# jserv/nstack

Hardware: AMD Instinct MI355X
Metric: device-resident CRC-32 FCS GiB/s on 1518-B frames, 1/2/4/8 MI355X; % HBM peak (higher is better)
Workload: dtype u8

## Files before the change

nstack_amd/csrc/fcs_engine.cpp:

```cpp
#include <hip/hip_runtime.h>

#include <algorithm>
#include <atomic>
#include <cerrno>
#include <cstdarg>
#include <cstdio>
#include <cstdlib>
#include <chrono>
#include <cstring>
#include <map>
#include <memory>
#include <mutex>
#include <set>
#include <string>
#include <thread>
#include <vector>
#include <initializer_list>

#include "../../include/nstack_fcs.h"
#include "fcs_device.hpp"
#include "fcs_error.hpp"
#include "fcs_host_crc.hpp"
#include "fcs_launch.hpp"
#include "fcs_tables.hpp"
// ... 1447 lines not shown
    if (ds->tx_flag) hipHostFree(ds->tx_flag);
    if (ds->tx_dcount) hipFree(ds->tx_dcount);
    if (ds->vz_off) hipHostFree(ds->vz_off);
    if (ds->vz_len) hipHostFree(ds->vz_len);
    if (ds->vz_ok) hipHostFree(ds->vz_ok);
    if (ds->vz_dbad) hipFree(ds->vz_dbad);
    if (ds->one_stream) hipStreamDestroy(ds->one_stream);
    if (ds->one_h) hipHostFree(ds->one_h);
    if (ds->one_hout) hipHostFree(ds->one_hout);
    if (ds->one_flag) hipHostFree(ds->one_flag);
    for (DevState::OneLane &L : ds->one_lane) {
        if (L.st) hipStreamDestroy(L.st);
        if (L.flag) hipHostFree(L.flag);
    }
    if (!ds->q_streams.empty() || !ds->q_host.empty() || !ds->q_dev.empty()) (void)device_sync();
    for (hipStream_t q : ds->q_streams) hipStreamDestroy(q);
    for (void *h : ds->q_host) hipHostFree(h);
    for (void *d : ds->q_dev) hipFree(d);
    for (hipEvent_t ev : ds->ctr_done)
        if (ev) hipEventDestroy(ev);
    if (ds->d_blob) hipFree(ds->d_blob);
    if (ds->d_one_blob) hipFree(ds->d_one_blob);
    if (ds->d_kinit) hipFree(ds->d_kinit);
    if (ds->d_ctr) hipFree(ds->d_ctr);
    for (uint32_t *scr : ds->ctr_scr)
        if (scr) hipFree(scr);
}

extern "C" {

const char *fcs_last_error(void) { return g_last_error.c_str(); }

const char *fcs_engine_version(void) {
    return "nstack-fcs 0.6 gfx950: quarter-wave/frame, 96B lane windows as 2 slice-by-4 chains, v_perm "
           "addressing, DPP reduce; 1496-1524B: LDS-DMA (nt global_load_lds) 6KiB slot/wave, 16 waves/CU, "
           "32KiB 8-replica tables, guided dynamic items; 130-399B: 4 lanes x 36-104B, 400-868B: 8 lanes x 44-112B windows/frame, 870-1476B: 16 lanes x 60-96B windows, 6-7KiB LDS-DMA slots; <=128B: lane/frame; 1477-1495B, 1525-1988B: 104/120/128B-window LDS-DMA, 7/8KiB slots; "
           ">1524B otherwise: frame-interleaved LDS-DMA segments of 900-1988B (least m*(WD+8)); var: "
           "packed 64-1536B units as an arena stream (4KiB LDS-DMA items, taps at frame boundaries, XOR "
           "scan), other units as a flat chunk stream per 64-frame window";
}

int fcs_engine_init(int ndev) {
    int total = 0;
    hipError_t e = hipGetDeviceCount(&total);
    if (e != hipSuccess || total <= 0) return fail(ENODEV, "no HIP device visible (%s)", hipGetErrorString(e));
    const int use = ndev <= 0 ? total : ((ndev > total && !alias_devices_enabled()) ? total : ndev);
    {
        std::lock_guard<std::mutex> lk(g_mu);
        g_engine_devs.clear();
        for (int d = 0; d < use; d++) g_engine_devs.push_back(d);
        for (auto it = g_alias.begin(); it != g_alias.end();) {
            if (it->first >= use) {
                g_alias_retired.push_back(std::move(it->second));
                it = g_alias.erase(it);
            } else {
                ++it;
            }
        }
    }
    std::vector<DevState *> devs;
    int rc = engine_devices(&devs);
    if (rc) return rc;
    return use;
}

void fcs_engine_fini(void) {
    std::lock_guard<std::mutex> lk(g_mu);
    int cur = 0;
    (void)hipGetDevice(&cur);
    for (auto &up : g_dev)
        if (up) destroy_state(up.get());
    for (auto &kv : g_alias)
// ... 447 lines not shown
```

nstack_amd/csrc/fcs_kernel.hip:

```cpp
#include <hip/hip_runtime.h>
#include <stdint.h>

#include <atomic>

#include "dispenser.hpp"
#include "fcs_launch.hpp"
#include "fcs_tables.hpp"
#include "fcs_crc.hpp"
#include "wave_sync.hpp"

namespace fcs {

struct Item {
    uint64_t end;
    uint32_t len;
    uint32_t m;
};

template <bool VAR>
__device__ __forceinline__ Item frame_item(const KParams &p, uint64_t f) {
    Item it;
    if (VAR) {
        const uint32_t L = p.len[f];
        it.end = p.base + (p.off ? p.off[f] : f * p.stride) + L;
// ... 1514 lines not shown
#ifdef FCS_SHORT_NO_PIPE
    constexpr bool kPipe = false;
#else
    constexpr bool kPipe = W <= 24;
#endif
    if constexpr (!kPipe) {
        for (uint64_t it = D.first(); it != kEnd; it = D.next(it)) {
            Win x;
            load(it, x);
            crc(it, x);
        }
    } else {
    Win xa, xb;
    uint64_t it = D.first();
    if (it != kEnd) load(it, xa);
    while (it != kEnd) {
        const uint64_t i1 = D.next(it);
        if (i1 != kEnd) load(i1, xb);
        crc(it, xa);
        if (i1 == kEnd) break;
        const uint64_t i2 = D.next(i1);
        if (i2 != kEnd) load(i2, xa);
        crc(i1, xb);
        it = i2;
    }
    }
    flush_bad<kWideBad>(p, lds);
}

constexpr uint32_t kStChunk = 64;
constexpr uint32_t kStItem = 64 * kStChunk;
constexpr uint32_t kStSlotBytes = kStItem;
constexpr int kStWaves = kWgThreads / 64;
constexpr uint32_t kStHoleChunk = 0;
constexpr uint32_t kStHoleWord = kStHoleChunk + 4 * kStChunkTabs;
constexpr uint32_t kStHoleInv = kStHoleWord + 4 * kStWordTabs;
constexpr uint32_t kStHoleK1 = kStHoleInv + 4 * kStInvTabs;
constexpr uint32_t kStHoleMark = kStHoleK1 + 2;
constexpr uint32_t kStBad = dma_hole(kStHoleMark + 2 * 16);
static_assert(kStHoleMark + 2 * 16 + 1 <= 256, "holes");
static_assert(kStWaves <= 16, "marks and counters for 16 waves");
constexpr uint32_t kStSlots = 65536;
constexpr uint32_t kStRings = kStSlots + 16 * kStSlotBytes;
constexpr uint32_t kStLdsBytes = kStRings + 16 * 1024;
static_assert(kStLdsBytes <= 163840, "LDS per CU");
constexpr uint32_t kMarkStart = 1u << 31, kMarkEnd = 1u << 30;
constexpr uint32_t kStLenBits = 11;
static_assert(kStUnitFrames * kStMaxLen + 128 < (1u << (32 - kStLenBits)) && kStMaxLen < (1u << kStLenBits), "packing");
#ifdef FCS_STAMPS
#define ST_T(v)                              \
    __builtin_amdgcn_sched_barrier(0);       \
    const uint64_t v = __builtin_amdgcn_s_memtime(); \
    __builtin_amdgcn_sched_barrier(0);
#else
#define ST_T(v)
#endif
#ifndef FCS_ST_CHAINS
#define FCS_ST_CHAINS 1
#endif
#ifndef FCS_ST_AUX
#define FCS_ST_AUX 2
#endif
#ifndef FCS_ST_EDGE_AUX
#ifdef FCS_ST_ALIGN16
#define FCS_ST_EDGE_AUX 0
#else
#define FCS_ST_EDGE_AUX FCS_ST_AUX
#endif
#endif

#ifndef FCS_ST_NOSKEW
constexpr uint32_t kStSkew = 1;
#else
constexpr uint32_t kStSkew = 0;
#endif
__device__ __forceinline__ uint32_t hole_shift(const uint8_t *lds, uint32_t s, uint32_t h, uint32_t extra) {
    uint32_t r[8];
    const uint32_t base = h * 256u + kDmaHole;
    const uint32_t ev = 64u * ((h >> 2) & kStSkew), od = 64u - ev;
#pragma unroll
    for (int t = 0; t < 8; t++) {
        const uint32_t sh = (4 * t >= 2) ? (s >> (4 * t - 2)) : (s << 2);
        r[t] = lds_rd(lds, base + 256u * (uint32_t)(t >> 1) + ((t & 1) ? od : ev) + (sh & 0x3Cu));
    }
    return xor9(r, extra);
}

__device__ __forceinline__ uint32_t wave_xor_scan(uint32_t v) {
    v ^= (uint32_t)__builtin_amdgcn_update_dpp(0, (int)v, 0x111, 0xF, 0xF, true);
    v ^= (uint32_t)__builtin_amdgcn_update_dpp(0, (int)v, 0x112, 0xF, 0xF, true);
    v ^= (uint32_t)__builtin_amdgcn_update_dpp(0, (int)v, 0x114, 0xF, 0xF, true);
    v ^= (uint32_t)__builtin_amdgcn_update_dpp(0, (int)v, 0x118, 0xF, 0xF, true);
    v ^= (uint32_t)__builtin_amdgcn_update_dpp(0, (int)v, 0x142, 0xA, 0xF, false);
    v ^= (uint32_t)__builtin_amdgcn_update_dpp(0, (int)v, 0x143, 0xC, 0xF, false);
    return v;
}

__device__ __forceinline__ void stage_stream_tables(const KParams &p, uint8_t *lds, int tid) {
    for (int i = tid; i < 2048; i += kWgThreads) {
        const uint32_t v = p.blob[kBlobSlice + 256 * (3 - ((i & 7) >> 1)) + (i >> 3)];
        u32x4 vv = {v, v, v, v};
        *reinterpret_cast<u32x4 *>(lds + (uint32_t)(i >> 3) * 256u + (uint32_t)(i & 7) * 16u) = vv;
    }
    for (int i = tid; i < (kStChunkTabs + kStWordTabs + kStInvTabs) * 128; i += kWgThreads) {
        const uint32_t q = (uint32_t)i >> 7, t = ((uint32_t)i >> 4) & 7u, e = (uint32_t)i & 15u;
        *reinterpret_cast<uint32_t *>(lds + dma_hole(4u * q + (t >> 1)) + 64u * ((t + (q & kStSkew)) & 1u) + 4u * e) =
            p.blob[kBlobStream + i];
    }
    for (int i = tid; i < 64; i += kWgThreads)
        *reinterpret_cast<uint32_t *>(lds + dma_hole(kStHoleK1 + (uint32_t)i / 32u) + ((uint32_t)i % 32u) * 4u) =
            p.blob[kBlobStreamK1 + i];
    for (int i = tid; i < 2 * 16 * 32; i += kWgThreads)
        *reinterpret_cast<uint32_t *>(lds + dma_hole(kStHoleMark + (uint32_t)i / 32u) + ((uint32_t)i % 32u) * 4u) = 0u;
    for (int i = tid; i < 16 * 256; i += kWgThreads) reinterpret_cast<uint32_t *>(lds + kStRings)[i] = 0u;
}

template <int kQ>
__device__ __forceinline__ bool unit_unpacked(const KParams &p, uint64_t f0, uint32_t nf, int lane, uint64_t (&S)[kQ],
                                              uint32_t (&Ln)[kQ]) {
#pragma unroll
    for (int q = 0; q < kQ; q++) {
        const uint32_t g = 64u * (uint32_t)q + (uint32_t)lane;
        S[q] = g < nf ? p.off[f0 + g] : 0ull;
        Ln[q] = g < nf ? p.len[f0 + g] : kStMinLen;
    }
    bool bad = false;
#pragma unroll
    for (int q = 0; q < kQ; q++) {
        const uint32_t g = 64u * (uint32_t)q + (uint32_t)lane;
        bad |= Ln[q] < kStMinLen || Ln[q] > kStMaxLen;
        uint32_t nlo = (uint32_t)__shfl_down((int)(uint32_t)S[q], 1), nhi = (uint32_t)__shfl_down((int)(uint32_t)(S[q] >> 32), 1);
        if (q + 1 < kQ) {
            const uint32_t blo = (uint32_t)__builtin_amdgcn_readfirstlane((int)(uint32_t)S[q + 1]);
            const uint32_t bhi = (uint32_t)__builtin_amdgcn_readfirstlane((int)(uint32_t)(S[q + 1] >> 32));
            if (lane == 63) {
                nlo = blo;
                nhi = bhi;
            }
        }
        const uint64_t ns = ((uint64_t)nhi << 32) | nlo;
        bad |= g + 1 < nf && ns != S[q] + Ln[q];
    }
    return bad;
}

template <bool LOAD>
__global__ __launch_bounds__(kWgThreads, 1) void fcs_stream_kernel(KParams p) {
    __shared__ __attribute__((aligned(16))) uint8_t lds[kStLdsBytes];
    const int tid = threadIdx.x;
    stage_stream_tables(p, lds, tid);
    init_bad<kStBad>(lds);
    __syncthreads();

    const int lane = tid & 63;
    const uint32_t wave = (uint32_t)__builtin_amdgcn_readfirstlane(tid >> 6);
    const uint32_t h = (uint32_t)(lane >> 3) & 3u, r4 = (uint32_t)(lane & 7) * 4u;
    const uint32_t B[4] = {r4 + 32u * (0u ^ h), r4 + 32u * (1u ^ h), r4 + 32u * (2u ^ h), r4 + 32u * (3u ^ h)};
    const uint32_t SEL[4] = {0x0C0C0400u + ((0u ^ h) << 8), 0x0C0C0400u + ((1u ^ h) << 8),
                             0x0C0C0400u + ((2u ^ h) << 8), 0x0C0C0400u + ((3u ^ h) << 8)};
    uint8_t *slot = lds + kStSlots + wave * kStSlotBytes;
    uint32_t *acc = reinterpret_cast<uint32_t *>(lds + kStRings + wave * 1024u);
    uint32_t *tap = acc + 128;
    const uint32_t mark_lane = dma_hole(kStHoleMark + 2u * wave + ((uint32_t)lane >> 5)) + ((uint32_t)lane & 31u) * 4u;
    auto mark_at = [&](uint32_t c) {
        return reinterpret_cast<uint32_t *>(lds + dma_hole(kStHoleMark + 2u * wave + (c >> 5)) + (c & 31u) * 4u);
    };
    auto k1_of = [&](uint32_t sg) { return lds_rd(lds, dma_hole(kStHoleK1 + sg / 32u) + (sg % 32u) * 4u); };
    const uint32_t goff = 64u * ((uint32_t)lane >> 2) + 16u * (((uint32_t)lane - ((uint32_t)lane >> 4)) & 3u);
    const uint64_t hi16 = (p.hi4 + 15) & ~15ull;
    auto dma_item = [&](uint64_t X) {
        typedef __attribute__((address_space(3))) void lds_void;
        const uint64_t a = X + goff;
        lds_void *ls = (lds_void *)slot;
        if (X + kStItem <= hi16) {
            __builtin_amdgcn_global_load_lds(reinterpret_cast<const void *>(a), ls, 16, 0, FCS_ST_EDGE_AUX);
            __builtin_amdgcn_global_load_lds(reinterpret_cast<const void *>(a), ls, 16, 1024, FCS_ST_AUX);
            __builtin_amdgcn_global_load_lds(reinterpret_cast<const void *>(a), ls, 16, 2048, FCS_ST_AUX);
            __builtin_amdgcn_global_load_lds(reinterpret_cast<const void *>(a), ls, 16, 3072, FCS_ST_EDGE_AUX);
        } else {
            if (a < hi16) __builtin_amdgcn_global_load_lds(reinterpret_cast<const void *>(a), ls, 16, 0, FCS_ST_EDGE_AUX);
            if (a + 1024 < hi16) __builtin_amdgcn_global_load_lds(reinterpret_cast<const void *>(a), ls, 16, 1024, FCS_ST_AUX);
            if (a + 2048 < hi16) __builtin_amdgcn_global_load_lds(reinterpret_cast<const void *>(a), ls, 16, 2048, FCS_ST_AUX);
            if (a + 3072 < hi16) __builtin_amdgcn_global_load_lds(reinterpret_cast<const void *>(a), ls, 16, 3072, FCS_ST_EDGE_AUX);
        }
    };
    const uint32_t cbase = 64u * (uint32_t)lane, sw = ((uint32_t)lane >> 2) & 3u;
    const u32x4 *pc[4] = {reinterpret_cast<const u32x4 *>(slot + cbase + 16u * ((0u + sw) & 3u)),
                          reinterpret_cast<const u32x4 *>(slot + cbase + 16u * ((1u + sw) & 3u)),
                          reinterpret_cast<const u32x4 *>(slot + cbase + 16u * ((2u + sw) & 3u)),
                          reinterpret_cast<const u32x4 *>(slot + cbase + 16u * ((3u + sw) & 3u))};
    constexpr int kQ = (int)(kStUnitFrames / 64);
    constexpr uint32_t kLenMask = (1u << kStLenBits) - 1u;

    constexpr uint64_t kEnd = Dispenser::kEnd;
    const uint64_t units = (p.n + kStUnitFrames - 1) / kStUnitFrames;
#ifdef FCS_STAMPS
    uint64_t sts[8] = {0, 0, 0, 0, 0, 0, 0, 0};
    const uint64_t st_begin = __builtin_amdgcn_s_memtime();
#endif
    Dispenser D(p.ctr, units, (uint64_t)gridDim.x * kStWaves, (uint64_t)blockIdx.x * kStWaves + wave, lane, 100, 1, 8);
    uint32_t lx = 0;
#if defined(FCS_ST_PROBE_LDS) || defined(FCS_ST_PROBE_VALU)
    uint32_t probe = 0;
#endif
    for (uint64_t u = D.first(); u != kEnd; u = D.next(u)) {
        ST_T(tu0)
        const uint64_t f0 = u * kStUnitFrames;
        const uint32_t nf = (uint32_t)((p.n - f0) < kStUnitFrames ? (p.n - f0) : kStUnitFrames);
        uint64_t S[kQ];
        uint32_t Ln[kQ];
        const bool bad = unit_unpacked(p, f0, nf, lane, S, Ln);
        if (__any(bad)) {
            if (!LOAD && lane == 0) p.ulist[atomicAdd(p.ucount, 1u)] = (uint32_t)u;
            continue;
        }
        const uint64_t s0 = p.base + (((uint64_t)(uint32_t)__builtin_amdgcn_readfirstlane((int)(uint32_t)(S[0] >> 32)) << 32) |
                                      (uint32_t)__builtin_amdgcn_readfirstlane((int)(uint32_t)S[0]));
#ifdef FCS_ST_ALIGN16
        const uint64_t X0 = s0 & ~15ull;
#else
        const uint64_t lo16 = p.lo4 & ~15ull;
        const uint64_t X0 = (s0 & ~127ull) > lo16 ? (s0 & ~127ull) : lo16;
#endif
        dma_item(X0);
        const uint64_t o0 = X0 - p.base;
        const uint32_t last = nf - 1;
        uint32_t pk[kQ];
#pragma unroll
        for (int q = 0; q < kQ; q++) pk[q] = ((uint32_t)(S[q] + Ln[q] - o0) << kStLenBits) | Ln[q];
        uint32_t E = 0;
#pragma unroll
        for (int q = 0; q < kQ; q++)
            if ((last >> 6) == (uint32_t)q) E = (uint32_t)__builtin_amdgcn_readlane((int)pk[q], (int)(last & 63u)) >> kStLenBits;
        uint32_t cb = 0;
        const uint32_t nitems = (E + kStItem - 1) / kStItem;
#ifdef FCS_STAMPS
        {
            ST_T(tu1)
            sts[0] += tu1 - tu0;
            sts[6]++;
        }
#endif
        uint32_t nsf = 0, base_cnt = 0, closed = 0;
        uint32_t tend = 0;
        auto close_pass = [&](uint32_t b, uint32_t cnt, uint32_t pw) {
            wave_lds_sync();
            const uint32_t g = 64u * b + (uint32_t)lane;
            const uint32_t e = pw >> kStLenBits, L = pw & kLenMask;
            const uint32_t st = e - L, ss = st & 63u, se = e & 63u;
            const uint32_t Ts = tap[g & 127u];
            const uint32_t Te = g < last ? tap[(g + 1u) & 127u] : tend;
            const uint32_t a0 = acc[g & 127u];
            wave_lds_sync();
            acc[g & 127u] = 0u;
#ifdef FCS_ST_ABL_NOCLOSE
            const uint32_t reg = Ts ^ Te ^ a0 ^ k1_of(ss) ^ se;
#else
            const uint32_t U = hole_shift(lds, Ts, kStHoleWord + 4u * (15u - (ss >> 2)), k1_of(ss));
            const uint32_t js = (uint32_t)lane < cnt ? (e >> 6) - (st >> 6) - 1u : 0u;
            const uint32_t a = hole_shift(lds, U, kStHoleChunk + 4u * js, a0);
            const uint32_t inner = hole_shift(lds, a, kStHoleWord + 4u * ((se >> 2) + 1u), Te);
            const uint32_t reg = hole_shift(lds, inner, kStHoleInv + 4u * (3u - (se & 3u)), 0u);
#endif
            emit<kStBad>(p, lds, (uint32_t)lane < cnt, f0 + g, ~reg);
        };
        if (LOAD) {
            for (uint32_t t = 0; t < nitems; t++) {
                const uint32_t Xr = kStItem * t;
                __builtin_amdgcn_s_waitcnt(0x0F70);
#pragma unroll
                for (int i = 0; i < 4; i++) {
                    const u32x4 x = *pc[i];
                    lx ^= x.x ^ x.y ^ x.z ^ x.w;
                }
                __builtin_amdgcn_s_waitcnt(0xC07F);
                if (t + 1 < nitems) dma_item(X0 + Xr + kStItem);
            }
            wave_lds_sync();
            continue;
        }
        for (uint32_t t = 0; t < nitems; t++) {
            const uint32_t Xr = kStItem * t;
            ST_T(ti0)
            const uint32_t gA = 64u * cb + (uint32_t)lane, gB = gA + 64u;
            const uint32_t eA = pk[0] >> kStLenBits, eB = pk[1] >> kStLenBits;
            const uint32_t sA = eA - (pk[0] & kLenMask), sB = eB - (pk[1] & kLenMask);
            const bool inA = gA >= nsf && gA < nf && sA < Xr + kStItem;
            const bool inB = gB >= nsf && gB < nf && sB < Xr + kStItem;
            if (inA) *mark_at((sA - Xr) >> 6) = kMarkStart | (gA << 6) | ((sA - Xr) & 63u);
            if (inB) *mark_at((sB - Xr) >> 6) = kMarkStart | (gB << 6) | ((sB - Xr) & 63u);
            if (E < Xr + kStItem && lane == 0) *mark_at((E - Xr) >> 6) = kMarkEnd | ((E - Xr) & 63u);
            nsf += (uint32_t)__popcll(__ballot(inA)) + (uint32_t)__popcll(__ballot(inB));
            const uint32_t gl = nsf - 1u;
            const uint32_t el = (uint32_t)__builtin_amdgcn_readlane((int)((gl >> 6) == cb ? eA : eB), (int)(gl & 63u));
            const uint32_t le_far = (el - Xr) >> 6;
            wave_lds_sync();
            const uint32_t mk = lds_rd(lds, mark_lane);
            *reinterpret_cast<uint32_t *>(lds + mark_lane) = 0u;
            const bool isst = (mk & kMarkStart) != 0, isend = (mk & kMarkEnd) != 0;
            const uint32_t sig = mk & 63u, k = sig >> 2, r = sig & 3u, bf = (mk >> 6) & 1023u;
            const uint64_t Mst = __ballot(isst), Mend = __ballot(isend), Mb = Mst | Mend;
            const uint64_t upto = Mst & ((2ull << lane) - 1ull);
            const int o = (int)(base_cnt + (uint32_t)__popcll(upto)) - 1;
            const bool contrib = o >= 0 && Xr + 64u * (uint32_t)lane + 63u < E;
            const uint64_t after = lane == 63 ? 0ull : (Mb & (~0ull << (lane + 1)));
            const uint32_t le = after ? (uint32_t)__builtin_ctzll(after) : le_far;
            const uint32_t j = contrib ? le - (uint32_t)lane - 1u : 0u;

            ST_T(ti1)
            __builtin_amdgcn_s_waitcnt(0x0F70);
            ST_T(ti2)
#ifdef FCS_STAMPS
            sts[1] += ti1 - ti0;
            sts[2] += ti2 - ti1;
#endif
            uint32_t w[16];
#pragma unroll
            for (int i = 0; i < 4; i++) {
                const u32x4 x = *pc[i];
                w[4 * i] = x.x;
                w[4 * i + 1] = x.y;
                w[4 * i + 2] = x.z;
                w[4 * i + 3] = x.w;
            }
            const uint32_t wk = lds_rd(slot, cbase + 16u * (((k >> 2) + sw) & 3u) + 4u * (k & 3u));
            __builtin_amdgcn_s_waitcnt(0xC07F);
            if (t + 1 < nitems) dma_item(X0 + Xr + kStItem);

            uint32_t x = w[0], xk = 0;
#ifdef FCS_ST_NOCRC
#pragma unroll
            for (int i = 1; i < 16; i++) x ^= w[i];
            xk = x ^ k;
#elif FCS_ST_CHAINS == 2
            uint32_t y = w[8];
#pragma unroll
            for (int i = 0; i < 8; i++) {
                if ((uint32_t)i == k) xk = x;
                if ((uint32_t)(i + 8) == k) xk = y;
                x = step4_l8(lds, x, i < 7 ? w[i + 1] : 0u, B, SEL);
                y = step4_l8(lds, y, i < 7 ? w[i + 9] : 0u, B, SEL);
            }
            const uint32_t c0 = x;
            x = hole_shift(lds, c0, kStHoleWord + 4u * 8u, y);
#else
#pragma unroll
            for (int i = 0; i < 16; i++) {
                if ((uint32_t)i == k) xk = x;
                x = step4_l8(lds, x, i < 15 ? w[i + 1] : 0u, B, SEL);
            }
#endif
#if FCS_ST_CHAINS == 2 && !defined(FCS_ST_NOCRC)
            const uint32_t Tp = hole_shift(lds, k >= 8u ? c0 : 0u, kStHoleWord + 4u * (k >= 8u ? k - 7u : 0u),
                                           step4_l8(lds, xk ^ (wk & (0xFFFFFFFFu << (8u * r))), 0u, B, SEL));
#else
            const uint32_t Tp = step4_l8(lds, xk ^ (wk & (0xFFFFFFFFu << (8u * r))), 0u, B, SEL);
#endif
            if (isst) tap[bf & 127u] = Tp;
            if (Mend) tend = (uint32_t)__builtin_amdgcn_readlane((int)Tp, (int)__builtin_ctzll(Mend));
#ifdef FCS_STAMPS
            ST_T(ti3)
            sts[3] += ti3 - ti2;
#endif

#ifdef FCS_ST_ABL_NOSHIFT
            const uint32_t Wc = x ^ j;
#elif defined(FCS_ST_SKIPJ0)
            uint32_t Wc = x;
            if (j) Wc = hole_shift(lds, x, kStHoleChunk + 4u * j, 0u);
#else
            const uint32_t Wc = hole_shift(lds, x, kStHoleChunk + 4u * j, 0u);
#endif
#ifdef FCS_ST_PROBE_LDS
#pragma unroll
            for (int i = 0; i < FCS_ST_PROBE_LDS; i++) probe ^= lds_rd(lds, ((uint32_t)lane & 31u) * 4u + (uint32_t)i * 256u);
#endif
#ifdef FCS_ST_PROBE_VALU
#pragma unroll
            for (int i = 0; i < FCS_ST_PROBE_VALU; i++) probe = xor3(probe, w[i & 15], (uint32_t)i) + (uint32_t)i;
#endif
            const uint32_t P = wave_xor_scan(contrib ? Wc : 0u);
            const int sl = upto ? 63 - __builtin_clzll(upto) : 0;
            const uint32_t Pb = (uint32_t)__shfl((int)P, sl > 0 ? sl - 1 : 0);
            const bool seg_end = lane == 63 || ((Mst >> (lane + 1)) & 1ull);
            const uint32_t v = P ^ (sl > 0 ? Pb : 0u);
            if (o >= 0 && seg_end && v) {
                uint32_t *ap = &acc[(uint32_t)o & 127u];
                *ap = *ap ^ v;
            }
            base_cnt += (uint32_t)__popcll(Mst);
            uint32_t ended = closed;
            if (Mst) ended = (uint32_t)__builtin_amdgcn_readlane((int)bf, 63 - __builtin_clzll(Mst));
            if (Mend) ended = nf;
            if (ended >= 64u * (cb + 1u) && 64u * (cb + 1u) <= last) {
                close_pass(cb, 64u, pk[0]);
                closed = 64u * (cb + 1u);
                cb++;
#pragma unroll
                for (int q = 0; q + 1 < kQ; q++) pk[q] = pk[q + 1];
            }
#ifdef FCS_STAMPS
            ST_T(ti4)
            sts[4] += ti4 - ti3;
            sts[5]++;
#endif
        }
        if (closed < nf) {
            if ((closed >> 6) == cb) close_pass(cb, nf - closed, pk[0]);
            else close_pass(cb + 1u, nf - closed, pk[1]);
            closed = nf;
        }
        wave_lds_sync();
    }
#ifdef FCS_STAMPS
    if (p.dbg != nullptr && lane == 0) {
        sts[7] = __builtin_amdgcn_s_memtime() - st_begin;
        const uint32_t wv = blockIdx.x * kStWaves + wave;
#pragma unroll
        for (int i = 0; i < 8; i++) p.dbg[wv * 8 + i] = sts[i];
    }
#endif
    if (LOAD) {
        if (lx == 0x5EEDF00Du && p.out) p.out[0] = lx;
        return;
    }
#if defined(FCS_ST_PROBE_LDS) || defined(FCS_ST_PROBE_VALU)
    if (probe == 0x5EEDF00Du && p.out) p.out[0] = probe;
#endif
    flush_bad<kStBad>(p, lds);
}

__device__ __forceinline__ uint64_t splitmix64(uint64_t x) {
    x += 0x9E3779B97F4A7C15ull;
    x = (x ^ (x >> 30)) * 0xBF58476D1CE4E5B9ull;
    x = (x ^ (x >> 27)) * 0x94D049BB133111EBull;
    return x ^ (x >> 31);
}

__global__ __launch_bounds__(256) void fill_splitmix_kernel(uint8_t *p, uint64_t bytes,
                                                            uint64_t seed, uint64_t off) {
    const uint64_t tid = (uint64_t)blockIdx.x * blockDim.x + threadIdx.x;
    const uint64_t nth = (uint64_t)gridDim.x * blockDim.x;
    const uint64_t head = (8 - (off & 7)) & 7;
// ... 456 lines not shown
```

nstack_amd/csrc/fcs_tables.hpp:

```cpp
#pragma once
#include <hip/hip_runtime.h>

#include <cstdint>
#include <cstring>
#include <vector>

namespace fcs {

constexpr uint32_t kPoly = 0xEDB88320u;
constexpr int kChunkBytes = 96;
constexpr int kChunkWords = kChunkBytes / 4;
constexpr int kGroup = 16;
constexpr int kSegBytes = kChunkBytes * kGroup;
constexpr int kJumpBytes = kSegBytes;

constexpr uint32_t kLdsData = 0;
constexpr uint32_t kLdsLane = 131072;
constexpr uint32_t kLdsJump = 147456;
constexpr uint32_t kLdsH48 = 147968;
constexpr uint32_t kLdsH24 = 148480;
constexpr uint32_t kLdsInv = 148992;
constexpr uint32_t kLdsM768 = 149376;
constexpr uint32_t kLdsWave = 149888;
constexpr uint32_t kLdsWaveBytes = 256;
// ... 12 lines not shown
constexpr uint32_t kDmaMinLen = 1496;
constexpr uint32_t kDmaItemBytes = 6144;
constexpr uint32_t kWideWin = 128;
__host__ __device__ constexpr uint32_t wide_win(int wd) { return 4u * (uint32_t)wd; }
__host__ __device__ constexpr uint32_t wide_step(int wd) { return 4u * (uint32_t)wd - 4u; }
__host__ __device__ constexpr uint32_t wide_cover(int wd) { return 15u * wide_step(wd) + wide_win(wd); }
__host__ __device__ constexpr uint32_t wide_slot(int wd) { return wd == 32 ? 8192u : (wd > 24 ? 7168u : 6144u); }
#ifndef FCS_WIDE_MID_WD_MIN
#define FCS_WIDE_MID_WD_MIN 15
#endif
constexpr int kWideMidMin = FCS_WIDE_MID_WD_MIN, kWideMidMax = 24;
static_assert(kWideMidMin >= 11 && kWideMidMin <= 20, "mid-length widths the launch switch instantiates");
__host__ __device__ constexpr bool wide_mid_ok(int wd) { return wd >= kWideMidMin && wd <= kWideMidMax && (wd - 1) % 4 != 0; }
constexpr int kWide8Min = 11, kWide8Max = 28;
__host__ __device__ constexpr uint32_t wide8_cover(int wd) { return 7u * wide_step(wd) + wide_win(wd); }
__host__ __device__ constexpr bool wide8_ok(int wd) { return wd >= kWide8Min && wd <= kWide8Max && (wd - 1) % 4 != 0; }
constexpr int kWide4Min = 9, kWide4Max = 26;
__host__ __device__ constexpr uint32_t wide4_cover(int wd) { return 3u * wide_step(wd) + wide_win(wd); }
__host__ __device__ constexpr bool wide4_ok(int wd) { return wd >= kWide4Min && wd <= kWide4Max && (wd - 1) % 16 != 0; }
constexpr uint32_t kWideCover = wide_cover(32);
constexpr uint32_t kWideCover26 = wide_cover(26);
constexpr uint32_t kWideCover30 = wide_cover(30);

constexpr uint32_t kBlobSlice = 0;
constexpr uint32_t kBlobLane = 1024;
constexpr uint32_t kBlobJump = kBlobLane + 8 * 16 * 32;
constexpr uint32_t kBlobH48 = kBlobJump + 8 * 16;
constexpr uint32_t kBlobH24 = kBlobH48 + 8 * 16;
constexpr uint32_t kBlobInv = kBlobH24 + 8 * 16;
constexpr uint32_t kBlobM768 = kBlobInv + kChunkBytes;
constexpr uint32_t kBlobFlat = kBlobM768 + 8 * 16;
constexpr uint32_t kBlobLaneDma = kBlobFlat + kFlatBytes / 4;
constexpr uint32_t kBlobMerge = kBlobLaneDma + 8 * 16 * 32;
constexpr int kStChunkTabs = 24, kStWordTabs = 17, kStInvTabs = 4;
constexpr uint32_t kBlobStream = kBlobMerge + 11 * 8 * 16;
constexpr uint32_t kBlobStreamK1 = kBlobStream + (kStChunkTabs + kStWordTabs + kStInvTabs) * 128;
constexpr uint32_t kBlobLaneWide = kBlobStreamK1 + 64;
constexpr uint32_t kBlobLaneWide26 = kBlobLaneWide + 8 * 16 * 32;
constexpr uint32_t kBlobLaneWide30 = kBlobLaneWide26 + 8 * 16 * 32;
constexpr uint32_t kBlobInvWide = kBlobLaneWide30 + 8 * 16 * 32;
constexpr uint32_t kBlobLaneMid = kBlobInvWide + kWideWin;
constexpr uint32_t kBlobLane8 = kBlobLaneMid + (kWideMidMax - kWideMidMin + 1) * 8 * 16 * 32;
constexpr uint32_t kBlobLane4 = kBlobLane8 + (kWide8Max - kWide8Min + 1) * 8 * 16 * 32;
constexpr uint32_t kBlobWords = kBlobLane4 + (kWide4Max - kWide4Min + 1) * 8 * 16 * 32;
static_assert((kLdsInv - kLdsLane) / 4 == kBlobInv - kBlobLane, "blob/LDS order");
static_assert((kLdsM768 - kLdsLane) / 4 == kBlobM768 - kBlobLane, "blob/LDS order");

struct Tables {
    uint32_t T[4][256];
    uint8_t top_inv[256];

    Tables() {
        for (uint32_t b = 0; b < 256; b++) {
            uint32_t r = b;
            for (int i = 0; i < 8; i++) r = (r >> 1) ^ ((r & 1u) ? kPoly : 0u);
            T[0][b] = r;
        }
        for (int k = 1; k < 4; k++)
            for (int b = 0; b < 256; b++)
                T[k][b] = (T[k - 1][b] >> 8) ^ T[0][T[k - 1][b] & 0xFF];
        for (int b = 0; b < 256; b++) top_inv[T[0][b] >> 24] = (uint8_t)b;
    }
    uint32_t zstep(uint32_t s) const { return (s >> 8) ^ T[0][s & 0xFF]; }
    uint32_t zunstep(uint32_t s) const {
        uint32_t i = top_inv[s >> 24];
        return ((s ^ T[0][i]) << 8) | i;
    }
    uint32_t shift(uint32_t s, long n) const {
        for (; n > 0; n--) s = zstep(s);
        for (; n < 0; n++) s = zunstep(s);
        return s;
    }
    void nibble_table(long n, uint32_t out[8][16]) const {
        uint32_t img[32];
        for (int b = 0; b < 32; b++) img[b] = shift(1u << b, n);
        for (int t = 0; t < 8; t++)
            for (int e = 0; e < 16; e++) {
// ... 17 lines not shown
            for (int e = 0; e < 16; e++) b[kBlobJump + t * 16 + e] = nt[t][e];
        nibble_table(48, nt);
        for (int t = 0; t < 8; t++)
            for (int e = 0; e < 16; e++) b[kBlobH48 + t * 16 + e] = nt[t][e];
        nibble_table(24, nt);
        for (int t = 0; t < 8; t++)
            for (int e = 0; e < 16; e++) b[kBlobH24 + t * 16 + e] = nt[t][e];
        for (int z = 0; z < kChunkBytes; z++) b[kBlobInv + z] = shift(0xFFFFFFFFu, -(long)z);
        nibble_table(-768, nt);
        for (int t = 0; t < 8; t++)
            for (int e = 0; e < 16; e++) b[kBlobM768 + t * 16 + e] = nt[t][e];
        for (int c = 0; c < 16; c++) {
            nibble_table((long)kChunkBytes * c, nt);
            for (int t = 0; t < 8; t++)
                for (int e = 0; e < 16; e++) b[kBlobFlat + c * (kFlatStride / 4) + t * 16 + e] = nt[t][e];
        }
        for (int slot = 0; slot < 32; slot++) {
            nibble_table((long)dma_end_off(slot % kGroup), nt);
            for (int t = 0; t < 8; t++)
                for (int e = 0; e < 16; e++) b[kBlobLaneDma + (t * 16 + e) * 32 + slot] = nt[t][e];
        }
        for (int k = 1; k <= 11; k++) {
            nibble_table(8L * k, nt);
            for (int t = 0; t < 8; t++)
                for (int e = 0; e < 16; e++) b[kBlobMerge + (k - 1) * 128 + t * 16 + e] = nt[t][e];
        }
        int q = 0;
        auto put = [&](long n) {
            nibble_table(n, nt);
            for (int t = 0; t < 8; t++)
                for (int e = 0; e < 16; e++) b[kBlobStream + q * 128 + t * 16 + e] = nt[t][e];
            q++;
        };
        for (int j = 0; j < kStChunkTabs; j++) put(64L * j);
        for (int i = 0; i < kStWordTabs; i++) put(4L * i);
        for (int d = 1; d <= kStInvTabs; d++) put(-(long)d);
        for (int sg = 0; sg < 64; sg++) b[kBlobStreamK1 + sg] = shift(0xFFFFFFFFu, 64 - sg);
        for (int slot = 0; slot < 32; slot++) {
            nibble_table((long)wide_step(32) * (slot % kGroup), nt);
            for (int t = 0; t < 8; t++)
                for (int e = 0; e < 16; e++) b[kBlobLaneWide + (t * 16 + e) * 32 + slot] = nt[t][e];
            nibble_table((long)wide_step(26) * (slot % kGroup), nt);
            for (int t = 0; t < 8; t++)
                for (int e = 0; e < 16; e++) b[kBlobLaneWide26 + (t * 16 + e) * 32 + slot] = nt[t][e];
            nibble_table((long)wide_step(30) * (slot % kGroup), nt);
            for (int t = 0; t < 8; t++)
                for (int e = 0; e < 16; e++) b[kBlobLaneWide30 + (t * 16 + e) * 32 + slot] = nt[t][e];
        }
        for (int z = 0; z < (int)kWideWin; z++) b[kBlobInvWide + z] = shift(0xFFFFFFFFu, -(long)z);
        for (int wd = kWideMidMin; wd <= kWideMidMax; wd++)
            for (int slot = 0; slot < 32; slot++) {
                nibble_table((long)wide_step(wd) * (slot % kGroup), nt);
                for (int t = 0; t < 8; t++)
                    for (int e = 0; e < 16; e++)
                        b[kBlobLaneMid + (wd - kWideMidMin) * 4096 + (t * 16 + e) * 32 + slot] = nt[t][e];
            }
        for (int wd = kWide8Min; wd <= kWide8Max; wd++)
            for (int slot = 0; slot < 32; slot++) {
                nibble_table((long)wide_step(wd) * (slot % 8), nt);
                for (int t = 0; t < 8; t++)
                    for (int e = 0; e < 16; e++) b[kBlobLane8 + (wd - kWide8Min) * 4096 + (t * 16 + e) * 32 + slot] = nt[t][e];
            }
        for (int wd = kWide4Min; wd <= kWide4Max; wd++)
            for (int slot = 0; slot < 32; slot++) {
                nibble_table((long)wide_step(wd) * (slot % 4), nt);
                for (int t = 0; t < 8; t++)
                    for (int e = 0; e < 16; e++) b[kBlobLane4 + (wd - kWide4Min) * 4096 + (t * 16 + e) * 32 + slot] = nt[t][e];
            }
        return b;
    }
// ... 15 lines not shown
```

Before: 6063.

## Use lane-fixed half-wave chunk shifts and per-frame inverse segment close in arena stream

Reworks the variable-length arena stream CRC path. Each lane's chunk CRC is now shifted by a fixed per-lane amount to the end of its half-wave, using a lane-indexed table, instead of a data-dependent distance. Frames are closed with a segment shift plus an inverse 2048-byte shift and new end-tail tables, and taps are stored raw without an extra step. This replaces per-item variable table lookups and shuffle/popcount bookkeeping with mbcnt/bpermute and select trees. The cost is a reorganised LDS table layout, a second accumulator bank per ring, and a more complex close pass.

```diff
diff --git a/nstack_amd/csrc/fcs_engine.cpp b/nstack_amd/csrc/fcs_engine.cpp
--- a/nstack_amd/csrc/fcs_engine.cpp
+++ b/nstack_amd/csrc/fcs_engine.cpp
@@ -1503,12 +1503,13 @@
 const char *fcs_last_error(void) { return g_last_error.c_str(); }
 
 const char *fcs_engine_version(void) {
-    return "nstack-fcs 0.6 gfx950: quarter-wave/frame, 96B lane windows as 2 slice-by-4 chains, v_perm "
+    return "nstack-fcs 0.7 gfx950: quarter-wave/frame, 96B lane windows as 2 slice-by-4 chains, v_perm "
            "addressing, DPP reduce; 1496-1524B: LDS-DMA (nt global_load_lds) 6KiB slot/wave, 16 waves/CU, "
            "32KiB 8-replica tables, guided dynamic items; 130-399B: 4 lanes x 36-104B, 400-868B: 8 lanes x 44-112B windows/frame, 870-1476B: 16 lanes x 60-96B windows, 6-7KiB LDS-DMA slots; <=128B: lane/frame; 1477-1495B, 1525-1988B: 104/120/128B-window LDS-DMA, 7/8KiB slots; "
            ">1524B otherwise: frame-interleaved LDS-DMA segments of 900-1988B (least m*(WD+8)); var: "
-           "packed 64-1536B units as an arena stream (4KiB LDS-DMA items, taps at frame boundaries, XOR "
-           "scan), other units as a flat chunk stream per 64-frame window";
+           "packed 64-1536B units as an arena stream (4KiB LDS-DMA items, raw taps at frame boundaries, "
+           "lane-fixed half-wave chunk shift, XOR scan, per-frame close with the inverse segment shift), "
+           "other units as a flat chunk stream per 64-frame window";
 }
 
 int fcs_engine_init(int ndev) {
diff --git a/nstack_amd/csrc/fcs_kernel.hip b/nstack_amd/csrc/fcs_kernel.hip
--- a/nstack_amd/csrc/fcs_kernel.hip
+++ b/nstack_amd/csrc/fcs_kernel.hip
@@ -1570,21 +1570,27 @@
 constexpr uint32_t kStItem = 64 * kStChunk;
 constexpr uint32_t kStSlotBytes = kStItem;
 constexpr int kStWaves = kWgThreads / 64;
-constexpr uint32_t kStHoleChunk = 0;
-constexpr uint32_t kStHoleWord = kStHoleChunk + 4 * kStChunkTabs;
-constexpr uint32_t kStHoleInv = kStHoleWord + 4 * kStWordTabs;
-constexpr uint32_t kStHoleK1 = kStHoleInv + 4 * kStInvTabs;
+constexpr uint32_t kStHoleLane = 0;
+constexpr uint32_t kStHoleWord = kStHoleLane + 128;
+constexpr uint32_t kStHoleByte = kStHoleWord + 4 * kStWordTabs;
+constexpr uint32_t kStHoleSeg = kStHoleByte + 4 * kStByteTabs;
+constexpr uint32_t kStHoleK1 = kStHoleSeg + 4 * kStSegTabs;
 constexpr uint32_t kStHoleMark = kStHoleK1 + 2;
 constexpr uint32_t kStBad = dma_hole(kStHoleMark + 2 * 16);
 static_assert(kStHoleMark + 2 * 16 + 1 <= 256, "holes");
+static_assert(kStHoleWord % 8 == 0, "hole_shift's skew takes the table's parity from its hole number");
 static_assert(kStWaves <= 16, "marks and counters for 16 waves");
 constexpr uint32_t kStSlots = 65536;
 constexpr uint32_t kStRings = kStSlots + 16 * kStSlotBytes;
-constexpr uint32_t kStLdsBytes = kStRings + 16 * 1024;
+constexpr uint32_t kStRingBytes = 3 * 128 * 4;
+constexpr uint32_t kStEnd = kStRings + 16 * kStRingBytes;
+constexpr uint32_t kStLdsBytes = kStEnd + kStEndTabs * 512;
 static_assert(kStLdsBytes <= 163840, "LDS per CU");
 constexpr uint32_t kMarkStart = 1u << 31, kMarkEnd = 1u << 30;
 constexpr uint32_t kStLenBits = 11;
 static_assert(kStUnitFrames * kStMaxLen + 128 < (1u << (32 - kStLenBits)) && kStMaxLen < (1u << kStLenBits), "packing");
+static_assert(kStItem == 1u << 12 && (kStUnitFrames * kStMaxLen + 128) / kStItem + 1 < (1u << (20 - kStLenBits)),
+              "a start's item number is start >> 12; the all-ones start lies in no item");
 #ifdef FCS_STAMPS
 #define ST_T(v)                              \
     __builtin_amdgcn_sched_barrier(0);       \
@@ -1620,6 +1626,18 @@
     for (int t = 0; t < 8; t++) {
         const uint32_t sh = (4 * t >= 2) ? (s >> (4 * t - 2)) : (s << 2);
         r[t] = lds_rd(lds, base + 256u * (uint32_t)(t >> 1) + ((t & 1) ? od : ev) + (sh & 0x3Cu));
+    }
+    return xor9(r, extra);
+}
+
+__device__ __forceinline__ uint32_t end_shift(const uint8_t *lds, uint32_t s, uint32_t q, uint32_t extra) {
+    uint32_t r[8];
+    const uint32_t base = kStEnd + q * 512u;
+    const uint32_t ev = 64u * (q & kStSkew), od = 64u - ev;
+#pragma unroll
+    for (int t = 0; t < 8; t++) {
+        const uint32_t sh = (4 * t >= 2) ? (s >> (4 * t - 2)) : (s << 2);
+        r[t] = lds_rd(lds, base + 128u * (uint32_t)(t >> 1) + ((t & 1) ? od : ev) + (sh & 0x3Cu));
     }
     return xor9(r, extra);
 }
@@ -1640,17 +1658,25 @@
         u32x4 vv = {v, v, v, v};
         *reinterpret_cast<u32x4 *>(lds + (uint32_t)(i >> 3) * 256u + (uint32_t)(i & 7) * 16u) = vv;
     }
-    for (int i = tid; i < (kStChunkTabs + kStWordTabs + kStInvTabs) * 128; i += kWgThreads) {
+    for (int i = tid; i < 4096; i += kWgThreads)
+        *reinterpret_cast<uint32_t *>(lds + dma_hole(kStHoleLane + ((uint32_t)i >> 5)) + (uint32_t)(i & 31) * 4u) =
+            p.blob[kBlobStreamLane + i];
+    for (int i = tid; i < kStHoleTabs * 128; i += kWgThreads) {
         const uint32_t q = (uint32_t)i >> 7, t = ((uint32_t)i >> 4) & 7u, e = (uint32_t)i & 15u;
-        *reinterpret_cast<uint32_t *>(lds + dma_hole(4u * q + (t >> 1)) + 64u * ((t + (q & kStSkew)) & 1u) + 4u * e) =
-            p.blob[kBlobStream + i];
+        *reinterpret_cast<uint32_t *>(lds + dma_hole(kStHoleWord + 4u * q + (t >> 1)) + 64u * ((t + (q & kStSkew)) & 1u) +
+                                      4u * e) = p.blob[kBlobStream + i];
+    }
+    for (int i = tid; i < kStEndTabs * 128; i += kWgThreads) {
+        const uint32_t q = (uint32_t)i >> 7, t = ((uint32_t)i >> 4) & 7u, e = (uint32_t)i & 15u;
+        *reinterpret_cast<uint32_t *>(lds + kStEnd + 512u * q + 128u * (t >> 1) + 64u * ((t + (q & kStSkew)) & 1u) + 4u * e) =
+            p.blob[kBlobStream + kStHoleTabs * 128 + i];
     }
     for (int i = tid; i < 64; i += kWgThreads)
         *reinterpret_cast<uint32_t *>(lds + dma_hole(kStHoleK1 + (uint32_t)i / 32u) + ((uint32_t)i % 32u) * 4u) =
             p.blob[kBlobStreamK1 + i];
     for (int i = tid; i < 2 * 16 * 32; i += kWgThreads)
         *reinterpret_cast<uint32_t *>(lds + dma_hole(kStHoleMark + (uint32_t)i / 32u) + ((uint32_t)i % 32u) * 4u) = 0u;
-    for (int i = tid; i < 16 * 256; i += kWgThreads) reinterpret_cast<uint32_t *>(lds + kStRings)[i] = 0u;
+    for (int i = tid; i < (int)(16 * kStRingBytes / 4); i += kWgThreads) reinterpret_cast<uint32_t *>(lds + kStRings)[i] = 0u;
 }
 
 template <int kQ>
@@ -1697,8 +1723,10 @@
     const uint32_t SEL[4] = {0x0C0C0400u + ((0u ^ h) << 8), 0x0C0C0400u + ((1u ^ h) << 8),
                              0x0C0C0400u + ((2u ^ h) << 8), 0x0C0C0400u + ((3u ^ h) << 8)};
     uint8_t *slot = lds + kStSlots + wave * kStSlotBytes;
-    uint32_t *acc = reinterpret_cast<uint32_t *>(lds + kStRings + wave * 1024u);
-    uint32_t *tap = acc + 128;
+    uint32_t *acc = reinterpret_cast<uint32_t *>(lds + kStRings + wave * kStRingBytes);
+    uint32_t *tap = acc + 256;
+    const uint32_t lanebase = kDmaHole + ((uint32_t)lane & 31u) * 4u;
+    auto seg_shift = [&](uint32_t s, uint32_t y) { return lane_shift_dma(lds, s, kDmaHole + y * 4u); };
     const uint32_t mark_lane = dma_hole(kStHoleMark + 2u * wave + ((uint32_t)lane >> 5)) + ((uint32_t)lane & 31u) * 4u;
     auto mark_at = [&](uint32_t c) {
         return reinterpret_cast<uint32_t *>(lds + dma_hole(kStHoleMark + 2u * wave + (c >> 5)) + (c & 31u) * 4u);
@@ -1729,6 +1757,8 @@
                           reinterpret_cast<const u32x4 *>(slot + cbase + 16u * ((3u + sw) & 3u))};
     constexpr int kQ = (int)(kStUnitFrames / 64);
     constexpr uint32_t kLenMask = (1u << kStLenBits) - 1u;
+    constexpr uint32_t kPkNone = (((1u << (32 - kStLenBits)) - 1u) << kStLenBits) | kStMinLen;
+    auto pk_end = [&](uint32_t w) { return (w >> kStLenBits) + (w & kLenMask); };
 
     constexpr uint64_t kEnd = Dispenser::kEnd;
     const uint64_t units = (p.n + kStUnitFrames - 1) / kStUnitFrames;
@@ -1749,7 +1779,14 @@
         uint32_t Ln[kQ];
         const bool bad = unit_unpacked(p, f0, nf, lane, S, Ln);
         if (__any(bad)) {
-            if (!LOAD && lane == 0) p.ulist[atomicAdd(p.ucount, 1u)] = (uint32_t)u;
+            if (!LOAD && lane == 0) {
+#if defined(__HIP_DEVICE_COMPILE__)
+                typedef const volatile __attribute__((address_space(4))) KParams KArgs;
+                KArgs *ka = (KArgs *)__builtin_amdgcn_kernarg_segment_ptr();
+                uint32_t *const ul = ka->ulist;
+                ul[atomicAdd(ka->ucount, 1u)] = (uint32_t)u;
+#endif
+            }
             continue;
         }
         const uint64_t s0 = p.base + (((uint64_t)(uint32_t)__builtin_amdgcn_readfirstlane((int)(uint32_t)(S[0] >> 32)) << 32) |
@@ -1765,11 +1802,12 @@
         const uint32_t last = nf - 1;
         uint32_t pk[kQ];
 #pragma unroll
-        for (int q = 0; q < kQ; q++) pk[q] = ((uint32_t)(S[q] + Ln[q] - o0) << kStLenBits) | Ln[q];
+        for (int q = 0; q < kQ; q++)
+            pk[q] = lane < (int)nf - 64 * q ? ((uint32_t)(S[q] - o0) << kStLenBits) | Ln[q] : kPkNone;
         uint32_t E = 0;
 #pragma unroll
         for (int q = 0; q < kQ; q++)
-            if ((last >> 6) == (uint32_t)q) E = (uint32_t)__builtin_amdgcn_readlane((int)pk[q], (int)(last & 63u)) >> kStLenBits;
+            if ((last >> 6) == (uint32_t)q) E = pk_end((uint32_t)__builtin_amdgcn_readlane((int)pk[q], (int)(last & 63u)));
         uint32_t cb = 0;
         const uint32_t nitems = (E + kStItem - 1) / kStItem;
 #ifdef FCS_STAMPS
@@ -1779,28 +1817,32 @@
             sts[6]++;
         }
 #endif
-        uint32_t nsf = 0, base_cnt = 0, closed = 0;
+        uint32_t nsf = 0;
         uint32_t tend = 0;
         auto close_pass = [&](uint32_t b, uint32_t cnt, uint32_t pw) {
             wave_lds_sync();
             const uint32_t g = 64u * b + (uint32_t)lane;
-            const uint32_t e = pw >> kStLenBits, L = pw & kLenMask;
-            const uint32_t st = e - L, ss = st & 63u, se = e & 63u;
+            const uint32_t st = pw >> kStLenBits, e = pk_end(pw);
+            const uint32_t ss = st & 63u, se = e & 63u;
             const uint32_t Ts = tap[g & 127u];
             const uint32_t Te = g < last ? tap[(g + 1u) & 127u] : tend;
-            const uint32_t a0 = acc[g & 127u];
+            const uint32_t l0 = acc[g & 127u], h0 = acc[128u + (g & 127u)];
             wave_lds_sync();
             acc[g & 127u] = 0u;
+            acc[128u + (g & 127u)] = 0u;
 #ifdef FCS_ST_ABL_NOCLOSE
-            const uint32_t reg = Ts ^ Te ^ a0 ^ k1_of(ss) ^ se;
+            const uint32_t reg = Ts ^ Te ^ l0 ^ h0 ^ k1_of(ss) ^ se;
 #else
-            const uint32_t U = hole_shift(lds, Ts, kStHoleWord + 4u * (15u - (ss >> 2)), k1_of(ss));
-            const uint32_t js = (uint32_t)lane < cnt ? (e >> 6) - (st >> 6) - 1u : 0u;
-            const uint32_t a = hole_shift(lds, U, kStHoleChunk + 4u * js, a0);
-            const uint32_t inner = hole_shift(lds, a, kStHoleWord + 4u * ((se >> 2) + 1u), Te);
-            const uint32_t reg = hole_shift(lds, inner, kStHoleInv + 4u * (3u - (se & 3u)), 0u);
-#endif
-            emit<kStBad>(p, lds, (uint32_t)lane < cnt, f0 + g, ~reg);
+            const uint32_t ls = st >> 6, cl = (e >> 6) - 1u;
+            const uint32_t U = hole_shift(lds, Ts, kStHoleWord + 4u * (16u - (ss >> 2)), k1_of(ss));
+            const uint32_t Ush = seg_shift(U, ls & 31u);
+            const bool one = (ls >> 5) == (cl >> 5);
+            const uint32_t tot = hole_shift(lds, h0 ^ (one ? Ush : 0u), kStHoleSeg, l0 ^ (one ? 0u : Ush));
+            const uint32_t a64 = seg_shift(tot, 31u - (cl & 31u));
+            const uint32_t inner = end_shift(lds, a64, se >> 2, Te);
+            const uint32_t reg = hole_shift(lds, inner, kStHoleByte + 4u * (se & 3u), 0u);
+#endif
+            emit<kStBad>(p, lds, (uint32_t)lane < cnt, u * kStUnitFrames + g, ~reg);
         };
         if (LOAD) {
             for (uint32_t t = 0; t < nitems; t++) {
@@ -1821,16 +1863,15 @@
             const uint32_t Xr = kStItem * t;
             ST_T(ti0)
             const uint32_t gA = 64u * cb + (uint32_t)lane, gB = gA + 64u;
-            const uint32_t eA = pk[0] >> kStLenBits, eB = pk[1] >> kStLenBits;
-            const uint32_t sA = eA - (pk[0] & kLenMask), sB = eB - (pk[1] & kLenMask);
-            const bool inA = gA >= nsf && gA < nf && sA < Xr + kStItem;
-            const bool inB = gB >= nsf && gB < nf && sB < Xr + kStItem;
-            if (inA) *mark_at((sA - Xr) >> 6) = kMarkStart | (gA << 6) | ((sA - Xr) & 63u);
-            if (inB) *mark_at((sB - Xr) >> 6) = kMarkStart | (gB << 6) | ((sB - Xr) & 63u);
+            const uint32_t sA = pk[0] >> kStLenBits, sB = pk[1] >> kStLenBits;
+            const bool inA = (sA >> 12) == t, inB = (sB >> 12) == t;
+            if (inA) *mark_at((sA >> 6) & 63u) = (kMarkStart | (gA << 6)) | (sA & 63u);
+            if (inB) *mark_at((sB >> 6) & 63u) = (kMarkStart | (gB << 6)) | (sB & 63u);
             if (E < Xr + kStItem && lane == 0) *mark_at((E - Xr) >> 6) = kMarkEnd | ((E - Xr) & 63u);
+            const uint32_t base_cnt = nsf;
             nsf += (uint32_t)__popcll(__ballot(inA)) + (uint32_t)__popcll(__ballot(inB));
             const uint32_t gl = nsf - 1u;
-            const uint32_t el = (uint32_t)__builtin_amdgcn_readlane((int)((gl >> 6) == cb ? eA : eB), (int)(gl & 63u));
+            const uint32_t el = pk_end((uint32_t)__builtin_amdgcn_readlane((int)((gl >> 6) == cb ? pk[0] : pk[1]), (int)(gl & 63u)));
             const uint32_t le_far = (el - Xr) >> 6;
             wave_lds_sync();
             const uint32_t mk = lds_rd(lds, mark_lane);
@@ -1838,12 +1879,19 @@
             const bool isst = (mk & kMarkStart) != 0, isend = (mk & kMarkEnd) != 0;
             const uint32_t sig = mk & 63u, k = sig >> 2, r = sig & 3u, bf = (mk >> 6) & 1023u;
             const uint64_t Mst = __ballot(isst), Mend = __ballot(isend), Mb = Mst | Mend;
-            const uint64_t upto = Mst & ((2ull << lane) - 1ull);
-            const int o = (int)(base_cnt + (uint32_t)__popcll(upto)) - 1;
+            const int o = (int)__builtin_amdgcn_mbcnt_hi((uint32_t)(Mst >> 32), __builtin_amdgcn_mbcnt_lo((uint32_t)Mst, base_cnt)) +
+                          (isst ? 0 : -1);
             const bool contrib = o >= 0 && Xr + 64u * (uint32_t)lane + 63u < E;
             const uint64_t after = lane == 63 ? 0ull : (Mb & (~0ull << (lane + 1)));
             const uint32_t le = after ? (uint32_t)__builtin_ctzll(after) : le_far;
-            const uint32_t j = contrib ? le - (uint32_t)lane - 1u : 0u;
+            const bool early = ((le - 1u) >> 5) != ((uint32_t)lane >> 5);
+            const uint64_t upto = (Mst | (1ull << 32)) & ((2ull << lane) - 1ull);
+            const uint32_t sl4 = upto ? 4u * (63u - (uint32_t)__builtin_clzll(upto)) : 0u;
+            const bool seg_end = (lane & 31) == 31 || ((Mst >> (lane + 1)) & 1ull);
+            constexpr uint32_t kNone = 0xFFFFFFFFu;
+            const uint32_t aoff = o >= 0 && seg_end ? (early ? 0u : 128u) + ((uint32_t)o & 127u) : kNone;
+            const uint32_t toff = isst ? bf & 127u : kNone;
+            const uint32_t cmask = contrib ? 0xFFFFFFFFu : 0u;
 
             ST_T(ti1)
             __builtin_amdgcn_s_waitcnt(0x0F70);
@@ -1882,32 +1930,39 @@
             const uint32_t c0 = x;
             x = hole_shift(lds, c0, kStHoleWord + 4u * 8u, y);
 #else
+            const bool kb0 = (k & 1u) != 0;
+            uint32_t h0 = 0, pr[8];
 #pragma unroll
             for (int i = 0; i < 16; i++) {
-                if ((uint32_t)i == k) xk = x;
+                if (i & 1) pr[i >> 1] = kb0 ? x : h0;
+                else h0 = x;
                 x = step4_l8(lds, x, i < 15 ? w[i + 1] : 0u, B, SEL);
             }
+            {
+                const bool kb1 = (k & 2u) != 0, kb2 = (k & 4u) != 0, kb3 = (k & 8u) != 0;
+                const uint32_t q0 = kb1 ? pr[1] : pr[0], q1 = kb1 ? pr[3] : pr[2], q2 = kb1 ? pr[5] : pr[4],
+                               q3 = kb1 ? pr[7] : pr[6];
+                const uint32_t lo2 = kb2 ? q1 : q0, hi2 = kb2 ? q3 : q2;
+                xk = kb3 ? hi2 : lo2;
+            }
 #endif
 #if FCS_ST_CHAINS == 2 && !defined(FCS_ST_NOCRC)
-            const uint32_t Tp = hole_shift(lds, k >= 8u ? c0 : 0u, kStHoleWord + 4u * (k >= 8u ? k - 7u : 0u),
-                                           step4_l8(lds, xk ^ (wk & (0xFFFFFFFFu << (8u * r))), 0u, B, SEL));
+            const uint32_t Tp = hole_shift(lds, k >= 8u ? c0 : 0u, kStHoleWord + 4u * (k >= 8u ? k - 8u : 0u),
+                                           xk ^ (wk & (0xFFFFFFFFu << (8u * r))));
 #else
-            const uint32_t Tp = step4_l8(lds, xk ^ (wk & (0xFFFFFFFFu << (8u * r))), 0u, B, SEL);
-#endif
-            if (isst) tap[bf & 127u] = Tp;
-            if (Mend) tend = (uint32_t)__builtin_amdgcn_readlane((int)Tp, (int)__builtin_ctzll(Mend));
+            const uint32_t Tp = xk ^ (wk & (0xFFFFFFFFu << (8u * r)));
+#endif
+            if (toff != kNone) tap[toff] = Tp;
+            if (E < Xr + kStItem) tend = (uint32_t)__builtin_amdgcn_readlane((int)Tp, (int)((E - Xr) >> 6));
 #ifdef FCS_STAMPS
             ST_T(ti3)
             sts[3] += ti3 - ti2;
 #endif
 
 #ifdef FCS_ST_ABL_NOSHIFT
-            const uint32_t Wc = x ^ j;
-#elif defined(FCS_ST_SKIPJ0)
-            uint32_t Wc = x;
-            if (j) Wc = hole_shift(lds, x, kStHoleChunk + 4u * j, 0u);
+            const uint32_t Wc = x ^ lanebase;
 #else
-            const uint32_t Wc = hole_shift(lds, x, kStHoleChunk + 4u * j, 0u);
+            const uint32_t Wc = lane_shift_dma(lds, x, lanebase);
 #endif
 #ifdef FCS_ST_PROBE_LDS
 #pragma unroll
@@ -1917,36 +1972,31 @@
 #pragma unroll
             for (int i = 0; i < FCS_ST_PROBE_VALU; i++) probe = xor3(probe, w[i & 15], (uint32_t)i) + (uint32_t)i;
 #endif
-            const uint32_t P = wave_xor_scan(contrib ? Wc : 0u);
-            const int sl = upto ? 63 - __builtin_clzll(upto) : 0;
-            const uint32_t Pb = (uint32_t)__shfl((int)P, sl > 0 ? sl - 1 : 0);
-            const bool seg_end = lane == 63 || ((Mst >> (lane + 1)) & 1ull);
-            const uint32_t v = P ^ (sl > 0 ? Pb : 0u);
-            if (o >= 0 && seg_end && v) {
-                uint32_t *ap = &acc[(uint32_t)o & 127u];
+            const uint32_t W0 = Wc & cmask;
+            const uint32_t P = wave_xor_scan(W0);
+            const uint32_t Pb = (uint32_t)__builtin_amdgcn_ds_bpermute((int)sl4, (int)(P ^ W0));
+            const uint32_t v = P ^ Pb;
+            if (aoff != kNone && v) {
+                uint32_t *ap = &acc[aoff];
                 *ap = *ap ^ v;
             }
-            base_cnt += (uint32_t)__popcll(Mst);
-            uint32_t ended = closed;
-            if (Mst) ended = (uint32_t)__builtin_amdgcn_readlane((int)bf, 63 - __builtin_clzll(Mst));
-            if (Mend) ended = nf;
-            if (ended >= 64u * (cb + 1u) && 64u * (cb + 1u) <= last) {
-                close_pass(cb, 64u, pk[0]);
-                closed = 64u * (cb + 1u);
+            const bool lastitem = t + 1 == nitems;
+            const uint32_t ended = lastitem ? nf : nsf - 1u;
+            for (;;) {
+                const bool full = ended >= 64u * (cb + 1u) && 64u * (cb + 1u) <= last;
+                if (!full && !(lastitem && 64u * cb < nf)) break;
+                close_pass(cb, full ? 64u : nf - 64u * cb, pk[0]);
+                if (!full) break;
                 cb++;
 #pragma unroll
                 for (int q = 0; q + 1 < kQ; q++) pk[q] = pk[q + 1];
+                pk[kQ - 1] = kPkNone;
             }
 #ifdef FCS_STAMPS
             ST_T(ti4)
             sts[4] += ti4 - ti3;
             sts[5]++;
 #endif
-        }
-        if (closed < nf) {
-            if ((closed >> 6) == cb) close_pass(cb, nf - closed, pk[0]);
-            else close_pass(cb + 1u, nf - closed, pk[1]);
-            closed = nf;
         }
         wave_lds_sync();
     }
diff --git a/nstack_amd/csrc/fcs_tables.hpp b/nstack_amd/csrc/fcs_tables.hpp
--- a/nstack_amd/csrc/fcs_tables.hpp
+++ b/nstack_amd/csrc/fcs_tables.hpp
@@ -68,9 +68,12 @@
 constexpr uint32_t kBlobFlat = kBlobM768 + 8 * 16;
 constexpr uint32_t kBlobLaneDma = kBlobFlat + kFlatBytes / 4;
 constexpr uint32_t kBlobMerge = kBlobLaneDma + 8 * 16 * 32;
-constexpr int kStChunkTabs = 24, kStWordTabs = 17, kStInvTabs = 4;
+constexpr int kStWordTabs = 17, kStByteTabs = 4, kStSegTabs = 1, kStEndTabs = 16;
+constexpr int kStHoleTabs = kStWordTabs + kStByteTabs + kStSegTabs;
+constexpr int kStTabSlots = 45;
+static_assert(kStHoleTabs + kStEndTabs <= kStTabSlots, "stream tables");
 constexpr uint32_t kBlobStream = kBlobMerge + 11 * 8 * 16;
-constexpr uint32_t kBlobStreamK1 = kBlobStream + (kStChunkTabs + kStWordTabs + kStInvTabs) * 128;
+constexpr uint32_t kBlobStreamK1 = kBlobStream + kStTabSlots * 128;
 constexpr uint32_t kBlobLaneWide = kBlobStreamK1 + 64;
 constexpr uint32_t kBlobLaneWide26 = kBlobLaneWide + 8 * 16 * 32;
 constexpr uint32_t kBlobLaneWide30 = kBlobLaneWide26 + 8 * 16 * 32;
@@ -78,7 +81,8 @@
 constexpr uint32_t kBlobLaneMid = kBlobInvWide + kWideWin;
 constexpr uint32_t kBlobLane8 = kBlobLaneMid + (kWideMidMax - kWideMidMin + 1) * 8 * 16 * 32;
 constexpr uint32_t kBlobLane4 = kBlobLane8 + (kWide8Max - kWide8Min + 1) * 8 * 16 * 32;
-constexpr uint32_t kBlobWords = kBlobLane4 + (kWide4Max - kWide4Min + 1) * 8 * 16 * 32;
+constexpr uint32_t kBlobStreamLane = kBlobLane4 + (kWide4Max - kWide4Min + 1) * 8 * 16 * 32;
+constexpr uint32_t kBlobWords = kBlobStreamLane + 8 * 16 * 32;
 static_assert((kLdsInv - kLdsLane) / 4 == kBlobInv - kBlobLane, "blob/LDS order");
 static_assert((kLdsM768 - kLdsLane) / 4 == kBlobM768 - kBlobLane, "blob/LDS order");
 
@@ -162,10 +166,16 @@
                 for (int e = 0; e < 16; e++) b[kBlobStream + q * 128 + t * 16 + e] = nt[t][e];
             q++;
         };
-        for (int j = 0; j < kStChunkTabs; j++) put(64L * j);
         for (int i = 0; i < kStWordTabs; i++) put(4L * i);
-        for (int d = 1; d <= kStInvTabs; d++) put(-(long)d);
+        for (int r = 0; r < kStByteTabs; r++) put((long)r);
+        put(-2048L);
+        for (int i = 0; i < kStEndTabs; i++) put(4L * (i + 16));
         for (int sg = 0; sg < 64; sg++) b[kBlobStreamK1 + sg] = shift(0xFFFFFFFFu, 64 - sg);
+        for (int slot = 0; slot < 32; slot++) {
+            nibble_table(64L * (31 - slot), nt);
+            for (int t = 0; t < 8; t++)
+                for (int e = 0; e < 16; e++) b[kBlobStreamLane + (t * 16 + e) * 32 + slot] = nt[t][e];
+        }
         for (int slot = 0; slot < 32; slot++) {
             nibble_table((long)wide_step(32) * (slot % kGroup), nt);
             for (int t = 0; t < 8; t++)
```

Result: no change. 6070, median of 2 (+0.1%).
